# nikitinvv/libtike-cufft

Hardware: AMD Instinct MI355X
Metric: fwd+adj patterns/s (higher is better)
Workload: dtype f32

## Files before the change

libtike-cufft_amd/csrc/adjreg_map.hpp:

```cpp
#pragma once

namespace pty {

constexpr int kBucketPx = 4;

template <int N_, int NT_>
struct AdjRegCfg {
    static constexpr int N = N_, NT = NT_;
    static constexpr int C = 16;
    static constexpr int WC = C + kBucketPx;
    static constexpr int G = NT / WC;
    static constexpr int RPG = (N + G - 2) / (G - 1);
    static constexpr int HW = G * RPG;
    static constexpr int P = WC;
    static constexpr int COL0 = kBucketPx;
    static constexpr int TILE = (N + 2) * P + kBucketPx;
    static constexpr int SG = 1;
    static constexpr int STAGE = SG * RPG * WC;
    static_assert(G >= 2 && HW >= N + RPG, "window too low");
};

struct AdjRegWin {
    int t, X0, Ybase, gb;
};

template <class Cfg>
PTY_FN int adjreg_retire_count(const AdjRegWin& w, int t, int Xa, int sy) {
    const bool fits = t == w.t && Xa >= w.X0 && Xa + Cfg::C < w.X0 + Cfg::WC && sy >= w.Ybase && sy - w.Ybase < Cfg::HW;
    return fits ? (sy - w.Ybase) / Cfg::RPG : Cfg::G;
}

template <class Cfg>
PTY_FN void adjreg_advance(AdjRegWin& w, int nret, int t, int sx, int sy, int x0pad) {
    if (nret >= Cfg::G) {
        w.t = t;
        w.X0 = (sx / kBucketPx) * kBucketPx + x0pad;
        w.Ybase = sy;
        w.gb = 0;
    } else {
        w.Ybase += nret * Cfg::RPG;
        w.gb = (w.gb + nret) % Cfg::G;
    }
}

template <class Cfg>
PTY_FN int adjreg_rank(const AdjRegWin& w, int g) {
    const int k = g - w.gb;
    return k < 0 ? k + Cfg::G : k;
}
template <class Cfg>
PTY_FN int adjreg_row0(const AdjRegWin& w, int g) { return w.Ybase + adjreg_rank<Cfg>(w, g) * Cfg::RPG; }

template <class Cfg>
PTY_FN int adjreg_stage_slot(int rank, int r, int cw) { return (rank * Cfg::RPG + r) * Cfg::WC + cw; }

template <class Cfg>
PTY_FN int adjreg_tile_row(int i) {
    const int r = i + 1;
    return r < 0 ? 0 : (r > Cfg::N + 1 ? Cfg::N + 1 : r);
}

template <class Cfg>
PTY_FN void adjreg_combine(c32* acc, const c32* tile, const AdjRegWin& w, int g, int cw, int Xa, int sy, int pad, float fy, float fx) {
    constexpr int RPG = Cfg::RPG, P = Cfg::P;
    constexpr int B = 4, NB = (RPG + B - 1) / B;
    const float w00 = (1.0f - fx) * (1.0f - fy), w01 = fx * (1.0f - fy);
    const float w10 = (1.0f - fx) * fy, w11 = fx * fy;
    const int i0 = adjreg_row0<Cfg>(w, g) - sy + pad;
    const c32* tp = tile + (cw + Cfg::COL0 - 1 - (Xa - w.X0));
    const c32* tq = tp + adjreg_tile_row<Cfg>(i0 - 1) * P;
    c32 up0 = tq[1], up1 = tq[0];
    c32 t0[2][B], t1[2][B];
    auto request = [&](int b) {
#pragma unroll
        for (int u = 0; u < B; ++u) {
            if (b * B + u < RPG) {
                const c32* tr = tp + adjreg_tile_row<Cfg>(i0 + b * B + u) * P;
                t0[b & 1][u] = tr[1]; t1[b & 1][u] = tr[0];
            }
        }
        asm volatile("" ::: "memory");
    };
    request(0);
#pragma unroll
    for (int b = 0; b < NB; ++b) {
        if (b + 1 < NB) request(b + 1);
#pragma unroll
        for (int u = 0; u < B; ++u) {
            if (b * B + u < RPG) {
                acc[b * B + u] = acc[b * B + u] + (t0[b & 1][u] * w00 + t1[b & 1][u] * w01 + up0 * w10 + up1 * w11);
                up0 = t0[b & 1][u]; up1 = t1[b & 1][u];
            }
        }
    }
}

}
```

libtike-cufft_amd/csrc/k_cols_window.hpp:

```cpp
#pragma once


template <int N>
struct WinCfg {
    static constexpr int C = ColCfg<N>::C;
    static constexpr int WC = C + kBucketPx;
    static constexpr int H = N + 8;
    static constexpr bool fits = (size_t)((N + 2) * (C + 2) + H * WC) * sizeof(c32) <= 160 * 1024;
};

template <int N, bool SPLIT = false, int CW = 0>
__global__ __launch_bounds__(Plan<N>::T * (CW ? CW : ColCfg<N>::C)) void k_cols_adjwin(const ColArgs a, const int seglen) {
    using P = Plan<N>;
    using F = Fft<P, +1>;
    constexpr int E = P::E, T = P::T, C = CW ? CW : ColCfg<N>::C, NT = T * C;
    constexpr int LAST = P::NSTEP - 1;
    constexpr int WC = C + kBucketPx, H = WinCfg<N>::H;
    constexpr int CP = C + 2;
    __shared__ c32 lds[(N + 2) * CP];
    __shared__ c32 win[H * WC];

    const int tid = threadIdx.x;
    const int c = tid % C, j0 = tid / C;
    const int strip = blockIdx.x % a.nstrips, seg = blockIdx.x / a.nstrips;
    const int x0 = (a.strip0 + strip) * C;
    const int x = x0 + c;
    const Geom ge = a.ge;
    const int ix = x - ge.pad;
    const bool col_ok = ix >= 0 && ix < ge.nprb;
    const float cinv = 1.0f / (float)N;
    const c32 zero = c32{0.0f, 0.0f};
    const float det_sc = a.det_acc ? det_scale_of(a.det) : 0.0f;
    auto at = [&](int i) { return (i + 1) * CP + c + 1; };

    F fft;
    fft.init(j0, a.table);
    for (int o = tid; o < H * WC; o += NT) win[o] = zero;
    for (int o = tid; o < (N + 2) * CP; o += NT) lds[o] = zero;

    c32 pr[E];
    int cur_t = -1;
    int t_w = -1, X0 = 0, Ybase = 0, Ytop = 0;

    auto flush = [&](int ya, int yb) {
        if (yb <= ya) return;
        c32* fo = a.dst + (size_t)t_w * ge.nz * ge.n;
        const int cnt = (yb - ya) * WC;
        for (int o = tid; o < cnt; o += NT) {
            const int Y = ya + o / WC, col = o % WC;
            const int slot = (Y % H) * WC + col;
            const c32 v = win[slot];
            win[slot] = zero;
            const int X = X0 + col;
            if ((v.x != 0.0f || v.y != 0.0f) && Y < ge.nz && X >= 0 && X < ge.n) {
                const size_t e = ((size_t)t_w * ge.nz + Y) * ge.n + X;
                accum_c32(a.dst, a.det_acc, det_sc, e, v);
            }
        }
    };

    constexpr int NRG = NT / (C + 1) > 0 ? NT / (C + 1) : 1;
    constexpr int NITEM = (C + 1) * NRG;
    const int rpt = (ge.nprb + 1 + NRG - 1) / NRG;

    const RunBounds rb = run_bounds(a, seg, seglen);
    const int kb = rb.kb, ke = rb.ke;
    __shared__ RunMeta rm;
    load_run(rm, a.order, a.scan, kb, ke, tid);
    auto decode = [&](int k) { return run_decode(rm, k, kb, ke, ge); };
    auto tile_of = [&](const RunSt& st, int k) { return run_tile<N>(a, st.p, k); };

    __syncthreads();
    STAMP_DECL
    RunSt st = decode(kb);
    c32 v[E];
    if (st.have && st.q.valid) {
        const c32* tile_in = tile_of(st, kb);
        if (a.nt & 8)
            fft.template load<(SPLIT ? 1 : 0)>(v, j0, [&](int i) { return __builtin_nontemporal_load(tile_in + (size_t)i * N + x); });
        else
            fft.template load<(SPLIT ? 1 : 0)>(v, j0, [&](int i) { return tile_in[(size_t)i * N + x]; });
    }
    for (int k = kb; k < ke; ++k) {
        RunSt nx = decode(k + 1);
        if (!st.q.valid) {
            if (nx.have && nx.q.valid) {
                const c32* tile_in = tile_of(nx, k + 1);
                fft.template load<(SPLIT ? 1 : 0)>(v, j0, [&](int i) { return tile_in[(size_t)i * N + x]; });
            }
            st = nx;
            continue;
        }
        const Pos q = st.q;
        if (st.t != cur_t) {
            const c32* prb = a.aux + (size_t)st.t * ge.nprb * ge.nprb;
#pragma unroll
            for (int m = 0; m < E; ++m) {
                const int iy = j0 + m * T - ge.pad;
                const bool ok = col_ok && iy >= 0 && iy < ge.nprb;
                const c32 w = prb[ok ? ((size_t)iy * ge.nprb + ix) : 0];
                pr[m] = ok ? w * cinv : zero;
            }
            cur_t = st.t;
        }
        STAMP(0)
        STAMP_DRAIN();
        STAMP(1)
        if (SPLIT) {
            fft.template compute<LAST>(v);
        } else {
        fft.template compute<0>(v);
        if (P::NSTEP > 1) {
            fft.template store<0>(v, j0, [&](int i, c32 val) { lds[at(i)] = val; });
            __syncthreads();
            fft.template load<1>(v, j0, [&](int i) { return lds[at(i)]; });
            if (P::NSTEP > 2) {
                __syncthreads();
                fft.template compute<1>(v);
                fft.template store<1>(v, j0, [&](int i, c32 val) { lds[at(i)] = val; });
                __syncthreads();
                fft.template load<2>(v, j0, [&](int i) { return lds[at(i)]; });
            }
            fft.template compute<LAST>(v);
        }
        }
        {
            c32 nat[E];
            F::to_natural(v, nat);
#pragma unroll
            for (int m = 0; m < E; ++m) {
                const c32 w = pr[m];
                nat[m] = c32{w.x * nat[m].x + w.y * nat[m].y, w.x * nat[m].y - w.y * nat[m].x};
            }
            STAMP(2)
            if (SPLIT) __syncthreads();
            STAMP(3)
#pragma unroll
            for (int m = 0; m < E; ++m) lds[at(j0 + m * T)] = nat[m];
        }
        STAMP(8)
        if (nx.have && nx.q.valid) {
            const c32* tile_in = tile_of(nx, k + 1);
            if (a.nt & 8)
                fft.template load<(SPLIT ? 1 : 0)>(v, j0, [&](int i) { return __builtin_nontemporal_load(tile_in + (size_t)i * N + x); });
            else
                fft.template load<(SPLIT ? 1 : 0)>(v, j0, [&](int i) { return tile_in[(size_t)i * N + x]; });
        }
        STAMP(9)
        const int Xa = q.sx + x0 - ge.pad;
        const bool fitsw = (st.t == t_w) && Xa >= X0 && Xa + C < X0 + WC && q.sy >= Ybase;
        if (!fitsw) {
            __syncthreads();
            flush(Ybase, Ytop);
            t_w = st.t;
            X0 = (q.sx / kBucketPx) * kBucketPx + x0 - ge.pad;
            Ybase = q.sy;
            Ytop = q.sy;
        } else if (q.sy > Ybase) {
            flush(Ybase, q.sy < Ytop ? q.sy : Ytop);
            Ybase = q.sy;
            if (Ytop < Ybase) Ytop = Ybase;
        }
        if (Ytop < q.sy + ge.nprb + 1) Ytop = q.sy + ge.nprb + 1;
        STAMP(4)
        __syncthreads();
        STAMP(5)
        for (int item = tid; item < NITEM; item += NT) {
            const int cc = item % (C + 1), rg = item / (C + 1);
            const int ixo = x0 - ge.pad + cc;
            if (ixo < 0 || ixo > ge.nprb) continue;
            const float w00 = (1.0f - q.fx) * (1.0f - q.fy), w01 = q.fx * (1.0f - q.fy);
            const float w10 = (1.0f - q.fx) * q.fy, w11 = q.fx * q.fy;
            const int y0 = rg * rpt;
            int y1 = y0 + rpt;
            if (y1 > ge.nprb + 1) y1 = ge.nprb + 1;
            if (y0 >= y1) continue;
            const c32* tp = lds + (y0 + ge.pad) * CP + cc;
            c32 up0 = tp[1], up1 = tp[0];
            int slot = (q.sy + y0) % H;
            const int colw = Xa - X0 + cc;
            int yy = y0;
            auto trips = [&](auto uc) {
                constexpr int U = decltype(uc)::value;
                for (; yy + U <= y1; yy += U) {
                    c32 t0[U], t1[U], wv[U];
                    c32* wp[U];
#pragma unroll
                    for (int u = 0; u < U; ++u) {
                        const c32* tq = tp + (u + 1) * CP;
                        int su = slot + u;
                        su = su >= H ? su - H : su;
                        wp[u] = win + su * WC + colw;
                        t0[u] = tq[1]; t1[u] = tq[0];
                    }
#pragma unroll
                    for (int u = 0; u < U; ++u) wv[u] = *wp[u];
#pragma unroll
                    for (int u = 0; u < U; ++u) {
                        *wp[u] = wv[u] + (t0[u] * w00 + t1[u] * w01 + up0 * w10 + up1 * w11);
                        up0 = t0[u]; up1 = t1[u];
                    }
                    tp += U * CP;
                    slot += U;
                    slot = slot >= H ? slot - H : slot;
                }
            };
            trips(std::integral_constant<int, 3>{});
            for (; yy < y1; ++yy) {
                tp += CP;
                const c32 t00 = tp[1], t01 = tp[0];
                win[slot * WC + colw] += t00 * w00 + t01 * w01 + up0 * w10 + up1 * w11;
                up0 = t00; up1 = t01;
                slot = slot + 1 == H ? 0 : slot + 1;
            }
        }
        STAMP(6)
        if (!SPLIT) __syncthreads();
        st = nx;
    }
    __syncthreads();
    flush(Ybase, Ytop);
    STAMP(7)
    STAMP_FLUSH(a.stamps ? a.stamps + 12 : a.stamps)
}

template <int N, bool SPLIT = false>
__global__ __launch_bounds__(Plan<N>::T * ColCfg<N>::C, 2) void k_cols_adjreg(const ColArgs a, const int seglen) {
    using P = Plan<N>;
    using F = Fft<P, +1>;
    constexpr int E = P::E, T = P::T, C = ColCfg<N>::C, NT = T * C;
    constexpr int LAST = P::NSTEP - 1;
    using W = AdjRegCfg<N, NT>;
    static_assert(C == W::C, "strip width");
    constexpr int WC = W::WC, G = W::G, RPG = W::RPG;
    __shared__ c32 lds[W::TILE];
    __shared__ c32 wtab[N];
    __shared__ c32 stage[W::STAGE];

    const int tid = threadIdx.x;
    const int c = tid % C, j0 = tid / C;
    const int cw = tid % WC, g = tid / WC;
    const int strip = blockIdx.x % a.nstrips, seg = blockIdx.x / a.nstrips;
    const int x0 = (a.strip0 + strip) * C;
    const int x = x0 + c;
    const Geom ge = a.ge;
    const int ix = x - ge.pad;
    const bool col_ok = ix >= 0 && ix < ge.nprb;
    const float cinv = 1.0f / (float)N;
    const c32 zero = c32{0.0f, 0.0f};
    const float det_sc = a.det_acc ? det_scale_of(a.det) : 0.0f;
    auto at = [&](int i) { return (i + 1) * W::P + c + W::COL0; };

    F fft;
    for (int o = tid; o < N; o += NT) wtab[o] = a.table[o];
    for (int o = tid; o < W::TILE; o += NT) lds[o] = zero;

    c32 pr[E];
    int cur_t = -1;
    c32 acc[RPG];
#pragma unroll
    for (int r = 0; r < RPG; ++r) acc[r] = zero;
    AdjRegWin w{-1, 0, 0, 0};

    auto add_to_object = [&](const c32 v, int t, int Y, int X) {
        if ((v.x != 0.0f || v.y != 0.0f) && Y < ge.nz && X >= 0 && X < ge.n)
            accum_c32(a.dst, a.det_acc, det_sc, ((size_t)t * ge.nz + Y) * ge.n + X, v);
    };
    auto retire = [&](int nret) {
        if (w.t < 0 || g >= G || adjreg_rank<W>(w, g) >= nret) return;
        const int Y0 = adjreg_row0<W>(w, g), X = w.X0 + cw;
#pragma unroll
        for (int r = 0; r < RPG; ++r) {
            add_to_object(acc[r], w.t, Y0 + r, X);
            acc[r] = zero;
        }
    };
    auto stage_groups = [&](int nret) {
        if (g >= G) return;
        const int rank = adjreg_rank<W>(w, g);
        if (rank >= nret) return;
#pragma unroll
        for (int r = 0; r < RPG; ++r) {
            stage[adjreg_stage_slot<W>(rank, r, cw)] = acc[r];
            acc[r] = zero;
        }
    };

    const RunBounds rb = run_bounds(a, seg, seglen);
    const int kb = rb.kb, ke = rb.ke;
    __shared__ RunMeta rm;
    load_run(rm, a.order, a.scan, kb, ke, tid);
    auto decode = [&](int k) { return run_decode(rm, k, kb, ke, ge); };
    auto tile_of = [&](const RunSt& st, int k) { return run_tile<N>(a, st.p, k); };

    __syncthreads();
    STAMP_DECL
    RunSt st = decode(kb);
    c32 v[E];
    if (st.have && st.q.valid) {
        const c32* tile_in = tile_of(st, kb);
        if (a.nt & 8)
            fft.template load<(SPLIT ? 1 : 0)>(v, j0, [&](int i) { return __builtin_nontemporal_load(tile_in + (size_t)i * N + x); });
        else
            fft.template load<(SPLIT ? 1 : 0)>(v, j0, [&](int i) { return tile_in[(size_t)i * N + x]; });
    }
    for (int k = kb; k < ke; ++k) {
        RunSt nx = decode(k + 1);
        if (!st.q.valid) {
            if (nx.have && nx.q.valid) {
                const c32* tile_in = tile_of(nx, k + 1);
                fft.template load<(SPLIT ? 1 : 0)>(v, j0, [&](int i) { return tile_in[(size_t)i * N + x]; });
            }
            st = nx;
            continue;
        }
        const Pos q = st.q;
        int jz = j0;
        asm volatile("" : "+v"(jz));
        if (st.t != cur_t) {
            const c32* prb = a.aux + (size_t)st.t * ge.nprb * ge.nprb;
#pragma unroll
            for (int m = 0; m < E; ++m) {
                const int iy = j0 + m * T - ge.pad;
                const bool ok = col_ok && iy >= 0 && iy < ge.nprb;
                const c32 pw = prb[ok ? ((size_t)iy * ge.nprb + ix) : 0];
                pr[m] = ok ? pw * cinv : zero;
            }
            cur_t = st.t;
        }
        STAMP(0)
        STAMP_DRAIN();
        STAMP(1)
        if (SPLIT) {
            fft.template init_step<LAST>(jz, wtab);
            fft.template compute<LAST>(v);
        } else {
            fft.template compute<0>(v);
            if (P::NSTEP > 1) {
                fft.template store<0>(v, j0, [&](int i, c32 val) { lds[at(i)] = val; });
                __syncthreads();
                fft.template load<1>(v, j0, [&](int i) { return lds[at(i)]; });
                if (P::NSTEP > 2) {
                    __syncthreads();
                    if constexpr (P::NSTEP > 2) fft.template init_step<1>(jz, wtab);
                    fft.template compute<1>(v);
                    fft.template store<1>(v, j0, [&](int i, c32 val) { lds[at(i)] = val; });
                    __syncthreads();
                    fft.template load<2>(v, j0, [&](int i) { return lds[at(i)]; });
                }
                if constexpr (P::NSTEP > 1) fft.template init_step<LAST>(jz, wtab);
                fft.template compute<LAST>(v);
            }
        }
        {
            c32 nat[E];
            F::to_natural(v, nat);
#pragma unroll
            for (int m = 0; m < E; ++m) {
                const c32 pw = pr[m];
                nat[m] = c32{pw.x * nat[m].x + pw.y * nat[m].y, pw.x * nat[m].y - pw.y * nat[m].x};
            }
            STAMP(2)
            if (SPLIT) __syncthreads();
            STAMP(3)
#pragma unroll
            for (int m = 0; m < E; ++m) lds[at(j0 + m * T)] = nat[m];
        }
        STAMP(8)
        if (nx.have && nx.q.valid) {
            const c32* tile_in = tile_of(nx, k + 1);
            if (a.nt & 8)
                fft.template load<(SPLIT ? 1 : 0)>(v, j0, [&](int i) { return __builtin_nontemporal_load(tile_in + (size_t)i * N + x); });
            else
                fft.template load<(SPLIT ? 1 : 0)>(v, j0, [&](int i) { return tile_in[(size_t)i * N + x]; });
        }
        STAMP(9)
        const int Xa = q.sx + x0 - ge.pad;
        const int nret = adjreg_retire_count<W>(w, st.t, Xa, q.sy);
        const AdjRegWin was = w;
        int nstaged = 0;
        if (nret > 0) {
            if (nret <= W::SG) {
                stage_groups(nret);
                nstaged = nret;
            } else {
                retire(nret);
            }
            adjreg_advance<W>(w, nret, st.t, q.sx, q.sy, x0 - ge.pad);
        }
        STAMP(4)
        __syncthreads();
        STAMP(5)
        for (int o = tid; o < nstaged * RPG * WC; o += NT) add_to_object(stage[o], was.t, was.Ybase + o / WC, was.X0 + o % WC);
        if (g < G) adjreg_combine<W>(acc, lds, w, g, cw, Xa, q.sy, ge.pad, q.fy, q.fx);
        STAMP(6)
        if (!SPLIT) __syncthreads();
        st = nx;
    }
    retire(G);
    STAMP(7)
    STAMP_FLUSH(a.stamps ? a.stamps + 12 : a.stamps)
}

template <int N, int MODE, bool SPLIT = false, int NM = 1, int CW = 0>
__global__ __launch_bounds__(Plan<N>::T * (CW ? CW : ColCfg<N>::C)) void k_cols_gatherwin(const ColArgs a, const int seglen) {
    static_assert(MODE == M_FWD || MODE == M_ADJ_PRB, "forward operator or probe adjoint");
    static_assert(NM == 1 || (MODE == M_FWD && !SPLIT), "several probe modes: un-split forward pass only");
    if (MODE == M_FWD && a.skip && *a.skip != 0.0) return;
    using P = Plan<N>;
    constexpr int DIR = (MODE == M_FWD) ? -1 : +1;
    using F = Fft<P, DIR>;
    constexpr int E = P::E, T = P::T, C = CW ? CW : ColCfg<N>::C, NT = T * C;
    constexpr int LAST = P::NSTEP - 1;
    constexpr int WC = C + kBucketPx, H = WinCfg<N>::H;
    constexpr int R0 = P::radix(0);
    __shared__ c32 lds[SPLIT ? 1 : N * C];
    __shared__ c32 win[(H + 1) * WC];

    const int tid = threadIdx.x;
    const int c = tid % C, j0 = tid / C;
    const int strip = blockIdx.x % a.nstrips, seg = blockIdx.x / a.nstrips;
    const int x0 = (a.strip0 + strip) * C;
    const int x = x0 + c;
    const Geom ge = a.ge;
    const int ix = x - ge.pad;
    const bool col_ok = ix >= 0 && ix < ge.nprb;
    const float cinv = 1.0f / (float)N;
    const c32 zero = c32{0.0f, 0.0f};
    const float det_sc = (MODE == M_ADJ_PRB && a.det_acc) ? det_scale_of(a.det) : 0.0f;

    __shared__ c32 wtab[NM > 1 ? N : 1];
    F fft;
    if (NM == 1) fft.init(j0, a.table);
    else for (int o = tid; o < N; o += NT) wtab[o] = a.table[o];
    for (int o = tid; o < (H + 1) * WC; o += NT) win[o] = zero;

    c32 pr[E];
    c32 prnext[NM > 1 ? E : 1];
    int cur_t = -1;
    auto probe_strip = [&](c32* dst, int km, int t) {
        const c32* prb = (NM == 1 ? a.aux : a.auxm[km]) + (size_t)t * ge.nprb * ge.nprb;
#pragma unroll
        for (int b = 0; b < E / R0; ++b)
#pragma unroll
            for (int tt = 0; tt < R0; ++tt) {
                const int iy = j0 + b * T + tt * (N / R0) - ge.pad;
                const bool ok = col_ok && iy >= 0 && iy < ge.nprb;
                const c32 w = prb[ok ? ((size_t)iy * ge.nprb + ix) : 0];
                dst[b * R0 + tt] = ok ? w * cinv : zero;
            }
    };
    int t_w = -1, X0 = 0, Ylo = 0, Yhi = 0;

    auto flush_probe = [&](int t) {
#pragma unroll
        for (int m = 0; m < E; ++m) {
            const int iy = j0 + m * T - ge.pad;
            if (col_ok && iy >= 0 && iy < ge.nprb) {
                const size_t e = ((size_t)t * ge.nprb + iy) * ge.nprb + ix;
                accum_c32(a.dst, a.det_acc, det_sc, e, pr[m] * cinv);
            }
        }
    };

    const RunBounds rb = run_bounds(a, seg, seglen);
    const int kb = rb.kb, ke = rb.ke;
    __shared__ RunMeta rm;
    load_run(rm, a.order, a.scan, kb, ke, tid);

    struct St { int p, t, Xa; Pos q; bool have; };
    c32 pre_val = zero;
    int pre_slot = -1;
    bool pre_inb = false;
    auto prepare_issue = [&](int k, int kend) -> St {
        St st;
        st.have = k < kend;
        st.p = 0; st.t = 0; st.Xa = 0; st.q = Pos{0, 0, 0.f, 0.f, false, false};
        pre_slot = -1;
        if (!st.have) return st;
        st.p = uni_i(rm.p[k - kb]);
        st.t = st.p / ge.nscan;
        st.q = decode_xy(uni_f(rm.py[k - kb]), uni_f(rm.px[k - kb]), ge);
        if (!st.q.valid) return st;
        const c32* ft = (MODE == M_FWD ? a.src : a.aux) + (size_t)st.t * ge.nz * ge.n;
        st.Xa = st.q.sx + x0 - ge.pad;
        const int Ra = st.q.sy, Rb = st.q.sy + ge.nprb + 1;
        const bool colfit = (st.t == t_w) && st.Xa >= X0 && st.Xa + C < X0 + WC;
        if (!colfit) {
            t_w = st.t;
            X0 = (st.q.sx / kBucketPx) * kBucketPx + x0 - ge.pad;
            Ylo = Ra; Yhi = Ra;
        } else if (Ra < Ylo || Ra > Yhi) {
            Ylo = Ra; Yhi = Ra;
        } else {
            Ylo = Ra;
        }
        if (Rb > Yhi) {
            const int cnt = (Rb - Yhi) * WC;
            if (cnt <= NT) {
                if (tid < cnt) {
                    const int Y = Yhi + tid / WC, col = tid % WC;
                    const int X = X0 + col;
                    const bool inb = Y < ge.nz && X >= 0 && X < ge.n;
                    pre_val = ft[inb ? ((size_t)Y * ge.n + X) : 0];
                    pre_inb = inb;
                    pre_slot = (Y % H) * WC + col;
                }
            } else {
                for (int o = tid; o < cnt; o += NT) {
                    const int Y = Yhi + o / WC, col = o % WC;
                    const int X = X0 + col;
                    const bool inb = Y < ge.nz && X >= 0 && X < ge.n;
                    const c32 val = ft[inb ? ((size_t)Y * ge.n + X) : 0];
                    const int ws = (Y % H) * WC + col;
                    win[ws] = inb ? val : zero;
                    if (ws < WC) win[H * WC + ws] = inb ? val : zero;
                }
            }
            Yhi = Rb;
        }
        return st;
    };
    auto prepare_commit = [&]() {
        if (pre_slot >= 0) {
            const c32 val = pre_inb ? pre_val : zero;
            win[pre_slot] = val;
            if (pre_slot < WC) win[H * WC + pre_slot] = val;
        }
    };
    auto prepare = [&](int k, int kend) -> St {
        St st = prepare_issue(k, kend);
        prepare_commit();
        return st;
    };

    __syncthreads();
    if constexpr (MODE == M_ADJ_PRB) {
        auto decode_only = [&](int k) -> St {
            const RunSt d = run_decode<false>(rm, k, kb, ke, ge);
            return St{d.p, d.t, 0, d.q, d.have};
        };
        auto load_tile = [&](c32* v, const St& st, int k) {
            const c32* tile_in = run_tile<N>(a, st.p, k);
            fft.template load<(SPLIT ? 1 : 0)>(v, j0, [&](int i) { return tile_in[(size_t)i * N + x]; });
        };
        __syncthreads();
        St st = decode_only(kb);
        c32 v[E];
        if (st.have && st.q.valid) load_tile(v, st, kb);
        for (int k = kb; k < ke; ++k) {
            St nx = decode_only(k + 1);
            if (!st.q.valid) {
                if (nx.have && nx.q.valid) load_tile(v, nx, k + 1);
                st = nx;
                continue;
            }
            if (st.t != cur_t) {
                if (cur_t >= 0) flush_probe(cur_t);
#pragma unroll
                for (int m = 0; m < E; ++m) pr[m] = zero;
                cur_t = st.t;
            }
            if (!SPLIT) fft.template compute<0>(v);
            if (!SPLIT && P::NSTEP > 1) {
                fft.template store<0>(v, j0, [&](int i, c32 val) { lds[i * C + c] = val; });
                __syncthreads();
            } else {
                __syncthreads();
            }
            const St cur = prepare_issue(k, ke);
            if (SPLIT) {
                fft.template compute<LAST>(v);
            } else if (P::NSTEP > 1) {
                fft.template load<1>(v, j0, [&](int i) { return lds[i * C + c]; });
                if (P::NSTEP > 2) {
                    __syncthreads();
                    fft.template compute<1>(v);
                    fft.template store<1>(v, j0, [&](int i, c32 val) { lds[i * C + c] = val; });
                    __syncthreads();
                    fft.template load<2>(v, j0, [&](int i) { return lds[i * C + c]; });
                }
                fft.template compute<LAST>(v);
            }
            c32 nat[E];
            F::to_natural(v, nat);
            if (nx.have && nx.q.valid) load_tile(v, nx, k + 1);
            prepare_commit();
            __syncthreads();
            const Pos q = cur.q;
            const float w00 = (1.0f - q.fx) * (1.0f - q.fy), w01 = q.fx * (1.0f - q.fy);
            const float w10 = (1.0f - q.fx) * q.fy, w11 = q.fx * q.fy;
            const int colw = cur.Xa - X0 + c;
            int slot = (q.sy + j0 - ge.pad + 2 * H) % H;
#pragma unroll
            for (int m = 0; m < E; ++m) {
                const int iy = j0 + m * T - ge.pad;
                const bool ok = col_ok && iy >= 0 && iy < ge.nprb;
                const c32* r0 = win + slot * WC + colw;
                const c32 patch = r0[0] * w00 + r0[1] * w01 + r0[WC] * w10 + r0[WC + 1] * w11;
                const c32 term = cmulc(nat[m], patch);
                pr[m] += ok ? term : zero;
                slot += T;
                slot = slot >= H ? slot - H : slot;
            }
            st = nx;
        }
        if (cur_t >= 0) flush_probe(cur_t);
    } else {
        St st = prepare(kb, ke);
        __syncthreads();
        STAMP_DECL
        for (int k = kb; k < ke; ++k) {
            if (NM > 1 || st.t != cur_t) {
                probe_strip(pr, 0, st.t);
                cur_t = st.t;
            }
            if (!st.q.valid) {
#pragma unroll
                for (int km = 0; km < NM; ++km) {
                    c32* tile_out = (NM == 1 ? a.dst : a.dstm[km]) + (size_t)st.p * N * N;
#pragma unroll
                    for (int m = 0; m < E; ++m) tile_out[(size_t)(j0 + m * T) * N + x] = zero;
                }
                __syncthreads();
                st = prepare(k + 1, ke);
                __syncthreads();
                continue;
            }
            const Pos q = st.q;
            const float w00 = (1.0f - q.fx) * (1.0f - q.fy), w01 = q.fx * (1.0f - q.fy);
            const float w10 = (1.0f - q.fx) * q.fy, w11 = q.fx * q.fy;
            const int colw = st.Xa - X0 + c;
            const int slot0 = (q.sy + j0 - ge.pad + 2 * H) % H;
            auto patch_at = [&](int slot) {
                const c32* r0 = win + slot * WC + colw;
                return r0[0] * w00 + r0[1] * w01 + r0[WC] * w10 + r0[WC + 1] * w11;
            };

            c32 v[E];
            c32 vbase[NM > 1 ? E : 1];
            St nx;
            {
                STAMP(0)
                c32 nat[E];
                int slot = slot0;
#pragma unroll
                for (int m = 0; m < E; ++m) {
                    nat[m] = patch_at(slot);
                    slot += T;
                    slot = slot >= H ? slot - H : slot;
                }
                F::from_natural(nat, v);
#ifdef PTY_STAMPS
                asm volatile("s_waitcnt lgkmcnt(0)" ::: "memory");
#pragma unroll
                for (int s2 = 0; s2 < E; ++s2) asm volatile("" : "+v"(v[s2]));
#endif
                STAMP(1)
                if (NM > 1) {
#pragma unroll
                    for (int s2 = 0; s2 < E; ++s2) vbase[s2] = v[s2];
                }
#pragma unroll
                for (int s2 = 0; s2 < E; ++s2) v[s2] = cmul(pr[s2], v[s2]);
            }
            fft.template compute<0>(v);
            if (SPLIT) {
                c32* tile_out = a.dst + (size_t)st.p * N * N;
#ifdef PTY_STAMPS
#pragma unroll
                for (int s2 = 0; s2 < E; ++s2) asm volatile("" : "+v"(v[s2]));
#endif
                STAMP(2)
                fft.template store<0>(v, j0, [&](int i, c32 val) { tile_out[(size_t)i * N + x] = val; });
                STAMP(3)
                __syncthreads();
                STAMP(4)
                nx = prepare_issue(k + 1, ke);
                prepare_commit();
                STAMP(5)
                __syncthreads();
                STAMP(6)
                st = nx;
                continue;
            }
            int jz = j0;
            if (NM > 1) asm volatile("" : "+v"(jz));
#pragma unroll
            for (int km = 0; km < NM; ++km) {
                if (NM > 1) {
                    if (km > 0) {
#pragma unroll
                        for (int s2 = 0; s2 < E; ++s2) v[s2] = cmul(prnext[s2], vbase[s2]);
                        fft.template compute<0>(v);
                    }
                    if (km + 1 < NM) probe_strip(prnext, km + 1, st.t);
                }
                if (P::NSTEP > 1) {
                    STAMP(2)
                    fft.template store<0>(v, j0, [&](int i, c32 val) { lds[i * C + c] = val; });
                    STAMP(3)
                    __syncthreads();
                    STAMP(4)
                    if (km == 0) nx = prepare_issue(k + 1, ke);
                    fft.template load<1>(v, j0, [&](int i) { return lds[i * C + c]; });
                    if (P::NSTEP > 2) {
                        __syncthreads();
                        if constexpr (NM > 1 && P::NSTEP > 2) fft.template init_step<1>(jz, wtab);
                        fft.template compute<1>(v);
                        fft.template store<1>(v, j0, [&](int i, c32 val) { lds[i * C + c] = val; });
                        __syncthreads();
                        fft.template load<2>(v, j0, [&](int i) { return lds[i * C + c]; });
                    }
                    if constexpr (NM > 1 && P::NSTEP > 1) fft.template init_step<LAST>(jz, wtab);
                    fft.template compute<LAST>(v);
                } else if (km == 0) {
                    __syncthreads();
                    nx = prepare_issue(k + 1, ke);
                }
                STAMP(5)
                c32* tile_out = (NM == 1 ? a.dst : a.dstm[km]) + (size_t)st.p * N * N;
                if (a.nt & 4)
                    fft.template store<LAST>(v, j0, [&](int i, c32 val) { __builtin_nontemporal_store(val, tile_out + (size_t)i * N + x); });
                else
                    fft.template store<LAST>(v, j0, [&](int i, c32 val) { tile_out[(size_t)i * N + x] = val; });
// ... 138 lines not shown
```

libtike-cufft_amd/csrc/k_rows.hpp:

```cpp
#pragma once

template <bool WGSYNC, bool TWLDS, class P, int DIR, class Put, class Get>
__device__ __forceinline__ void row_steps(Fft<P, DIR>& fft, c32* v, const int j0, Put put, Get get, const int jz = 0,
                                          const c32* wtab = nullptr) {
    constexpr int T = P::T, LAST = P::NSTEP - 1;
    fft.template compute<0>(v);
    if constexpr (P::NSTEP > 1) {
        fft.template store<0>(v, j0, put);
        row_sync<T, WGSYNC>();
        fft.template load<1>(v, j0, get);
        if constexpr (P::NSTEP > 2) {
            row_sync<T, WGSYNC>();
            if constexpr (TWLDS) fft.template init_step<1>(jz, wtab);
            fft.template compute<1>(v);
            fft.template store<1>(v, j0, put);
            row_sync<T, WGSYNC>();
            fft.template load<2>(v, j0, get);
        }
        if constexpr (TWLDS) fft.template init_step<LAST>(jz, wtab);
        fft.template compute<LAST>(v);
    }
}

template <int N, int DIR>
__global__ __launch_bounds__(256) void k_rows(const RowArgs a) {
    using P = Plan<N>;
    using F = Fft<P, DIR>;
    using L = RowLds<N>;
    constexpr int E = P::E, T = P::T, B = 256 / T;
    constexpr int LAST = P::NSTEP - 1;
    __shared__ c32 lds[P::NSTEP > 1 ? B * L::FS : 1];

    const int tid = threadIdx.x;
    const int f = tid / T, j0 = tid % T;
    F fft;
    fft.init(j0, a.table);
    const c32 zero = c32{0.0f, 0.0f};
    const long long nb = (a.nrows + B - 1) / B;
    for (long long batch = blockIdx.x; batch < nb; batch += gridDim.x) {
        const long long r = batch * B + f;
        const bool ok = r < a.nrows;
        const long long tile = r / N;
        const c32* srow = a.src + (size_t)((a.tile_index && ok) ? (long long)a.tile_index[tile] : tile) * N * N + (size_t)(r % N) * N;
        c32* drow = a.dst + ((a.dst_indexed && a.tile_index && ok)
                                 ? (size_t)a.tile_index[tile] * N * N + (size_t)(r % N) * N
                                 : (size_t)r * N);
        c32 v[E];
        if (a.nt & 1)
            fft.template load<0>(v, j0, [&](int i) { return (ok && i >= a.xa && i < a.xb) ? __builtin_nontemporal_load(srow + i) : zero; });
        else
            fft.template load<0>(v, j0, [&](int i) { return (ok && i >= a.xa && i < a.xb) ? srow[i] : zero; });
        fft.template compute<0>(v);
        if (P::NSTEP > 1) {
            fft.template store<0>(v, j0, [&](int i, c32 val) { lds[L::at(f, i)] = val; });
            row_sync<T>();
            fft.template load<1>(v, j0, [&](int i) { return lds[L::at(f, i)]; });
            if (P::NSTEP > 2) {
                row_sync<T>();
                fft.template compute<1>(v);
                fft.template store<1>(v, j0, [&](int i, c32 val) { lds[L::at(f, i)] = val; });
                row_sync<T>();
                fft.template load<2>(v, j0, [&](int i) { return lds[L::at(f, i)]; });
            }
            fft.template compute<LAST>(v);
        }
        if (a.nt & 2)
            fft.template store<LAST>(v, j0, [&](int i, c32 val) {
                if (ok && i >= a.wa && i < a.wb) __builtin_nontemporal_store(val, drow + i);
            });
        else
            fft.template store<LAST>(v, j0, [&](int i, c32 val) {
                if (ok && i >= a.wa && i < a.wb) drow[i] = val;
            });
        if (P::NSTEP > 1) row_sync<T>();
    }
}

template <int N, int DIR>
__global__ __launch_bounds__(256) void k_rows_split(const RowArgs a) {
    static_assert(N == 256, "split row pass is written for the 16 x 16 plan");
    using P = Plan<N>;
    using F = Fft<P, DIR>;
    using L = RowLds<N>;
    constexpr int E = P::E, T = P::T, B = 256 / T;
    constexpr int LAST = P::NSTEP - 1;
    __shared__ c32 lds[B * L::FS];

    const int tid = threadIdx.x;
    const int f = tid / T, j0 = tid % T;
    F fft;
    fft.init(j0, a.table);
    auto put = [&](int i, c32 val) { lds[L::at(f, i)] = val; };
    auto get = [&](int i) { return lds[L::at(f, i)]; };
    const c32 zero = c32{0.0f, 0.0f};
    const long long nitems = (a.nrows / N) * 16;
    for (long long item = blockIdx.x; item < nitems; item += gridDim.x) {
        const long long tile = item / 16;
        const int jp = (int)(item % 16);
        const long long stile = a.tile_index ? (long long)a.tile_index[tile] : tile;
        const c32* sbase = a.src + (size_t)stile * N * N;
        c32* dbase = a.dst + (size_t)((a.dst_indexed && a.tile_index) ? stile : tile) * N * N;
        c32 v[E];
        if (DIR < 0) {
            const int x = tid;
            const bool colok = x >= a.xa && x < a.xb;
#pragma unroll
            for (int t = 0; t < 16; ++t) {
                const c32 val = __builtin_nontemporal_load(sbase + (size_t)(jp + 16 * t) * N + x);
                v[t] = colok ? val : zero;
            }
#pragma unroll
            for (int t = 1; t < 16; ++t) v[t] = cmul(v[t], a.table[(jp * t) & (N - 1)]);
            fft_reg<16, -1>(v);
#pragma unroll
            for (int t = 0; t < 16; ++t) lds[L::at(t, x)] = v[brev(t, 4)];
            __syncthreads();
            fft.template load<0>(v, j0, get);
            row_steps<false, false>(fft, v, j0, put, get);
            c32* drow = dbase + (size_t)(jp + 16 * f) * N;
            fft.template store<LAST>(v, j0, [&](int i, c32 val) { __builtin_nontemporal_store(val, drow + i); });
            __syncthreads();
        } else {
            const c32* srow = sbase + (size_t)(jp + 16 * f) * N;
            fft.template load<0>(v, j0, [&](int i) { return __builtin_nontemporal_load(srow + i); });
            fft.template compute<0>(v);
            fft.template store<0>(v, j0, put);
            row_sync<T>();
            fft.template load<1>(v, j0, get);
            fft.template compute<LAST>(v);
            row_sync<T>();
            fft.template store<LAST>(v, j0, put);
            __syncthreads();
            const int x = tid;
#pragma unroll
            for (int t = 0; t < 16; ++t) v[t] = lds[L::at(t, x)];
            fft_reg<16, +1>(v);
            if (x >= a.wa && x < a.wb) {
#pragma unroll
                for (int k1 = 0; k1 < 16; ++k1)
                    __builtin_nontemporal_store(v[brev(k1, 4)], dbase + (size_t)(16 * jp + k1) * N + x);
            }
            __syncthreads();
        }
    }
}

__device__ __forceinline__ float fsqrt(float x) { return __builtin_amdgcn_sqrtf(x); }
__device__ __forceinline__ float frcp(float x) { return __builtin_amdgcn_rcpf(x); }
__device__ __forceinline__ float flog2(float x) { return __builtin_amdgcn_logf(x); }
constexpr float kLn2 = 0.693147180559945309f;
enum CgModel { MODEL_GAUSSIAN = 0, MODEL_POISSON_ML = 1 };
__device__ __forceinline__ c32 pml_shift(const c32 d, const c32 dl) {
    return d - dl * c32{flog2(d.x + 1e-32f), flog2(d.y + 1e-32f)};
}
__device__ __forceinline__ c32 pml_term(const c32 x, const c32 dl, const c32 c) {
    const c32 ax = c32{fabsf(x.x), fabsf(x.y)};
    return (ax - c) - dl * c32{flog2(ax.x + 1e-32f), flog2(ax.y + 1e-32f)};
}
template <bool PML>
struct TrialTerm {
    c32 sd, dl, c;
    __device__ __forceinline__ explicit TrialTerm(const c32 d) {
        if constexpr (PML) {
            dl = d * kLn2;
            c = pml_shift(d, dl);
        } else {
            sd = c32{fsqrt(d.x), fsqrt(d.y)};
        }
    }
    __device__ __forceinline__ c32 operator()(const c32 x) const {
        if constexpr (PML) {
            return pml_term(x, dl, c);
        } else {
            const c32 df = c32{fsqrt(fabsf(x.x)), fsqrt(fabsf(x.y))} - sd;
            return df * df;
        }
    }
};

__device__ __forceinline__ c32 load_masked(const c32* __restrict__ p, unsigned m) {
    const c32 val = __builtin_nontemporal_load(p);
    return c32{__uint_as_float(__float_as_uint(val.x) & m), __uint_as_float(__float_as_uint(val.y) & m)};
}
__device__ __forceinline__ float load_masked(const float* __restrict__ p, unsigned m) {
    return __uint_as_float(__float_as_uint(__builtin_nontemporal_load(p)) & m);
}

enum RowEp { EP_STATS = 1, EP_PROJECT = 2, EP_LINESEARCH = 3, EP_CROSS = 6, EP_LINESEARCH_M = 7, EP_STATS_M = 8 };
constexpr int kMaxModes = 8;
constexpr int kMaxCand = 16;
constexpr int kLsGroupsRows = 7;

struct RowFusedArgs {
    const c32* s1;
    const c32* s2;
    c32* out;
    const float* data;
    const c32* table;
    long long nrows;
    double* sums;
    const double* ab;
    float gamma0;
    int ncand;
    int xa, xb;
    const float* inten;
    float* acc1;
    int first;
    const c32* sm[2 * kMaxModes];
    int nmodes;
    c32* ip;
    double* st;
    const double* gamma_dev;
    double* maxword;
    FoldBuf fold;
    int overwrite;
    int decide, decide_which, decide_gamma_word, decide_next;
    unsigned long long* best_zero;
    int nbest;
    const unsigned* mask;
};

__device__ inline void ls_decide_dev(double* __restrict__ st, const int which, const int gamma_word, const int next_ngroups) {
    if (st[PTYCHO_ST_LS_RESOLVED] != 0.0) return;
    const int ngroups = (int)st[PTYCHO_ST_LS_NGROUPS];
    const int ncand = (int)st[PTYCHO_ST_LS_NCAND];
    int tried = (int)st[PTYCHO_ST_LS_TRIED];
    double step = st[PTYCHO_ST_LS_GAMMA0];
    bool done = false;
    for (int grp = 0; grp < ngroups && !done; ++grp) {
        const double* c = st + PTYCHO_ST_COSTS + grp * (kMaxCand + 1);
        const float fp1 = (float)c[ncand];
        for (int j = 0; j < ncand; ++j) {
            if (!((float)c[j] > fp1)) {
                st[gamma_word] = 0.5 * step;
                st[PTYCHO_ST_HINT + which] = (double)(tried + j);
                done = true;
                break;
            }
            if (step < 1e-32) {
                st[gamma_word] = 0.0;
                st[PTYCHO_ST_HINT + which] = 14.0;
                st[PTYCHO_ST_LS_FAILED] += 1.0;
                done = true;
                break;
            }
            step *= 0.5;
        }
        if (!done) tried += ncand;
    }
    if (!done && next_ngroups == 0) {
        st[gamma_word] = 0.0;
        st[PTYCHO_ST_LS_FAILED] += 1.0;
        done = true;
    }
    st[PTYCHO_ST_LS_RESOLVED] = done ? 1.0 : 0.0;
    st[PTYCHO_ST_LS_TRIED] = (double)tried;
    st[PTYCHO_ST_LS_GAMMA0] = step;
    st[PTYCHO_ST_LS_NCAND] = (double)kMaxCand;
    st[PTYCHO_ST_LS_NGROUPS] = (double)next_ngroups;
}


template <int N, int EP>
constexpr int fused_min_waves() {
    if (!is_pow2(N)) return 1;
    return (N <= 512 && (EP == EP_LINESEARCH || EP == EP_LINESEARCH_M || EP == EP_PROJECT || EP == EP_CROSS)) ? 2
           : (N == 512 && (EP == EP_STATS || EP == EP_STATS_M)) ? 3 : 1;
}
template <>
constexpr int fused_min_waves<256, EP_STATS>() { return 4;
}
template <int N>
__global__ __launch_bounds__(256) void k_pack_mask(const unsigned char* __restrict__ m, unsigned* __restrict__ out,
                                                   unsigned* __restrict__ nmeasured) {
    using P = Plan<N>;
    static_assert(P::E <= 32, "one mask word per thread and row");
    const int w = blockIdx.x * 256 + threadIdx.x;
    if (w >= N * P::T) return;
    const int y = w / P::T, j0 = w % P::T;
    unsigned bits = 0u;
    for (int k = 0; k < P::E; ++k) bits |= (m[y * N + j0 + k * P::T] != 0 ? 1u : 0u) << k;
    out[w] = bits;
    if (bits) atomicAdd(nmeasured, (unsigned)__popc(bits));
}
__device__ __forceinline__ unsigned mask_bit(unsigned w, int k) { return (unsigned)((int)(w << (31 - k)) >> 31); }
__device__ __forceinline__ float and_f(float x, unsigned m) { return __uint_as_float(__float_as_uint(x) & m); }
__device__ __forceinline__ c32 and_c(c32 x, unsigned m) { return c32{and_f(x.x, m), and_f(x.y, m)}; }

template <int N, int EP, bool FW = false, bool MASK = false, int MODEL = MODEL_GAUSSIAN>
// ... 395 lines not shown
```

Measured before the change: 1.704 million.

## Stage split column-pass tiles into LDS ring via direct global-to-LDS loads

For the split adjoint column kernel, tiles are now fetched with global_load_lds_dwordx4 into a per-wave LDS ring and read back in FFT order, with the next tile's request issued right after the read. This replaces per-thread strided global loads, and a lighter waitcnt-plus-barrier replaces __syncthreads. The split path now runs compute<0> instead of the last step, drops the LDS twiddle table, and the row kernel gains an explicit twiddle multiply via readlane. A host-side checker validates the ring mapping. The inline asm that manipulates m0 is fragile, and the changed split FFT step order alters numerics structure.

```diff
diff --git a/libtike-cufft_amd/csrc/adjreg_map.hpp b/libtike-cufft_amd/csrc/adjreg_map.hpp
--- a/libtike-cufft_amd/csrc/adjreg_map.hpp
+++ b/libtike-cufft_amd/csrc/adjreg_map.hpp
@@ -95,4 +95,29 @@
     }
 }
 
+template <int N_>
+struct AdjRingCfg {
+    static constexpr int N = N_, C = 16, E = 16, T = N / E;
+    static constexpr int WAVE = 64, NW = T * C / WAVE;
+    static constexpr int JW = WAVE / C;
+    static constexpr int PIECES = 8;
+    static constexpr int PIECE = WAVE * 2;
+    static constexpr int SEG = PIECES * PIECE;
+    static constexpr int RING = NW * SEG;
+    static constexpr int ROW_STEP = (WAVE / 8 / JW) * T;
+    static_assert(RING == N * C && SEG == JW * E * C, "the ring holds one strip tile");
+};
+
+template <class R>
+PTY_FN int adjring_src_row(int wave, int i, int lane) {
+    const int rr = 8 * i + lane / 8;
+    return wave * R::JW + rr % R::JW + (rr / R::JW) * R::T;
 }
+template <class R>
+PTY_FN int adjring_src_col(int lane) { return 2 * (lane % 8); }
+template <class R>
+PTY_FN int adjring_dst_slot(int wave, int i, int lane) { return wave * R::SEG + i * R::PIECE + 2 * lane; }
+template <class R>
+PTY_FN int adjring_read_slot(int tid, int m) { return (tid / R::WAVE) * R::SEG + m * R::WAVE + tid % R::WAVE; }
+
+}
diff --git a/libtike-cufft_amd/csrc/host_adjdma.cpp b/libtike-cufft_amd/csrc/host_adjdma.cpp
--- /dev/null
+++ b/libtike-cufft_amd/csrc/host_adjdma.cpp
@@ -0,0 +1,65 @@
+#include <cstdint>
+#include <cstdio>
+#include <vector>
+
+#include "fft_core.hpp"
+#include "adjreg_map.hpp"
+
+using namespace pty;
+
+template <int N, int ST>
+static bool check(const char* name) {
+    using P = Plan<N>;
+    using F = Fft<P, +1>;
+    using R = AdjRingCfg<N>;
+    constexpr int C = R::C, NT = P::T * C;
+    static_assert(P::E == R::E && P::T == R::T, "the ring is cut for the plan's threads");
+    long long bad = 0;
+    const size_t scratch_base = 4096;
+    for (int strip = 0; strip < N / C; ++strip) {
+        const int x0 = strip * C;
+        std::vector<int> ring(R::RING, -1);
+        std::vector<int> requested(N * C, 0);
+        for (int wave = 0; wave < R::NW; ++wave)
+            for (int i = 0; i < R::PIECES; ++i)
+                for (int lane = 0; lane < R::WAVE; ++lane) {
+                    const int row = adjring_src_row<R>(wave, i, lane), col = adjring_src_col<R>(lane);
+                    const int slot = adjring_dst_slot<R>(wave, i, lane);
+                    if (row < 0 || row >= N || col < 0 || col + 1 >= C) { ++bad; continue; }
+                    const size_t src = scratch_base + ((size_t)row * N + x0 + col) * sizeof(c32);
+                    if (src % 16 != 0) ++bad;
+                    if (row != adjring_src_row<R>(wave, 0, lane) + i * R::ROW_STEP) ++bad;
+                    if (slot != wave * R::SEG + i * R::PIECE + 2 * lane) ++bad;
+                    if (slot < wave * R::SEG || slot + 1 >= (wave + 1) * R::SEG) { ++bad; continue; }
+                    for (int e = 0; e < 2; ++e) {
+                        if (ring[slot + e] != -1) ++bad;
+                        ring[slot + e] = row * C + col + e;
+                        ++requested[row * C + col + e];
+                    }
+                }
+        for (int e = 0; e < N * C; ++e)
+            if (requested[e] != 1) ++bad;
+        for (int tid = 0; tid < NT; ++tid) {
+            const int c = tid % C, j0 = tid / C;
+            F fft;
+            c32 rows[P::E];
+            fft.template load<ST>(rows, j0, [&](int i) { return c32{(float)i, 0.0f}; });
+            for (int m = 0; m < P::E; ++m) {
+                const int slot = adjring_read_slot<R>(tid, m);
+                if (slot < (tid / R::WAVE) * R::SEG || slot >= (tid / R::WAVE + 1) * R::SEG) { ++bad; continue; }
+                if (ring[slot] != (int)rows[m].x * C + c) ++bad;
+            }
+        }
+    }
+    std::printf("N=%d %s waves=%d requests=%d segment=%zu B ring=%zu B row_step=%d bad=%lld %s\n", N, name, R::NW, R::PIECES,
+                (size_t)R::SEG * sizeof(c32), (size_t)R::RING * sizeof(c32), R::ROW_STEP, bad, bad == 0 ? "ok" : "BAD");
+    return bad == 0;
+}
+
+int main() {
+    bool ok = true;
+    ok = check<256, 1>("split") && ok;
+    ok = check<256, 0>("unsplit") && ok;
+    std::printf("%s\n", ok ? "OK" : "FAIL");
+    return ok ? 0 : 1;
+}
diff --git a/libtike-cufft_amd/csrc/k_cols_window.hpp b/libtike-cufft_amd/csrc/k_cols_window.hpp
--- a/libtike-cufft_amd/csrc/k_cols_window.hpp
+++ b/libtike-cufft_amd/csrc/k_cols_window.hpp
@@ -11,6 +11,7 @@
 
 template <int N, bool SPLIT = false, int CW = 0>
 __global__ __launch_bounds__(Plan<N>::T * (CW ? CW : ColCfg<N>::C)) void k_cols_adjwin(const ColArgs a, const int seglen) {
+    static_assert(!SPLIT || N == 256, "split column pass is written for the 16 x 16 plan");
     using P = Plan<N>;
     using F = Fft<P, +1>;
     constexpr int E = P::E, T = P::T, C = CW ? CW : ColCfg<N>::C, NT = T * C;
@@ -107,7 +108,7 @@
         STAMP_DRAIN();
         STAMP(1)
         if (SPLIT) {
-            fft.template compute<LAST>(v);
+            fft.template compute<0>(v);
         } else {
         fft.template compute<0>(v);
         if (P::NSTEP > 1) {
@@ -233,8 +234,12 @@
     using W = AdjRegCfg<N, NT>;
     static_assert(C == W::C, "strip width");
     constexpr int WC = W::WC, G = W::G, RPG = W::RPG;
-    __shared__ c32 lds[W::TILE];
-    __shared__ c32 wtab[N];
+    static_assert(!SPLIT || N == 256, "split column pass is written for the 16 x 16 plan");
+    using R = AdjRingCfg<N>;
+    constexpr int RINGN = SPLIT ? R::RING : 0;
+    __shared__ __attribute__((aligned(SPLIT ? 16 : 8))) c32 ring_tile[RINGN + W::TILE];
+    c32* const lds = ring_tile + RINGN;
+    __shared__ c32 wtab[SPLIT ? 1 : N];
     __shared__ c32 stage[W::STAGE];
 
     const int tid = threadIdx.x;
@@ -252,8 +257,36 @@
     auto at = [&](int i) { return (i + 1) * W::P + c + W::COL0; };
 
     F fft;
-    for (int o = tid; o < N; o += NT) wtab[o] = a.table[o];
+    if constexpr (!SPLIT) {
+        for (int o = tid; o < N; o += NT) wtab[o] = a.table[o];
+    }
     for (int o = tid; o < W::TILE; o += NT) lds[o] = zero;
+
+    const int lane = tid % R::WAVE, wave = uni_i(tid / R::WAVE);
+    const unsigned ring_m0 = (unsigned)(size_t)ring_tile + (unsigned)(wave * R::SEG * (int)sizeof(c32));
+    const unsigned ring_voff =
+        (unsigned)((adjring_src_row<R>(wave, 0, lane) * N + x0 + adjring_src_col<R>(lane)) * (int)sizeof(c32));
+    const int ring_rd = adjring_read_slot<R>(tid, 0);
+    auto ring_request = [&](const c32* tile_in) {
+#pragma unroll
+        for (int i = 0; i < R::PIECES; ++i) {
+            const c32* sb = tile_in + (size_t)i * R::ROW_STEP * N;
+            const unsigned dst = ring_m0 + (unsigned)(i * R::PIECE * (int)sizeof(c32));
+            unsigned keep;
+            asm volatile("s_mov_b32 %0, m0\n\ts_mov_b32 m0, %3\n\ts_nop 0\n\tglobal_load_lds_dwordx4 %1, %2\n\ts_mov_b32 m0, %0"
+                         : "=&s"(keep) : "v"(ring_voff), "s"(sb), "s"(dst) : "memory");
+        }
+    };
+    auto ring_read = [&](c32* v) {
+#pragma unroll
+        for (int m = 0; m < E; ++m) v[m] = ring_tile[ring_rd + m * R::WAVE];
+        asm volatile("s_waitcnt lgkmcnt(0)" ::: "memory");
+    };
+    auto ring_barrier = [&]() {
+        asm volatile("s_waitcnt lgkmcnt(0)" ::: "memory");
+        __builtin_amdgcn_s_barrier();
+        asm volatile("" ::: "memory");
+    };
 
     c32 pr[E];
     int cur_t = -1;
@@ -299,17 +332,22 @@
     c32 v[E];
     if (st.have && st.q.valid) {
         const c32* tile_in = tile_of(st, kb);
-        if (a.nt & 8)
-            fft.template load<(SPLIT ? 1 : 0)>(v, j0, [&](int i) { return __builtin_nontemporal_load(tile_in + (size_t)i * N + x); });
-        else
-            fft.template load<(SPLIT ? 1 : 0)>(v, j0, [&](int i) { return tile_in[(size_t)i * N + x]; });
+        if constexpr (SPLIT) {
+            ring_request(tile_in);
+        } else {
+            if (a.nt & 8)
+                fft.template load<0>(v, j0, [&](int i) { return __builtin_nontemporal_load(tile_in + (size_t)i * N + x); });
+            else
+                fft.template load<0>(v, j0, [&](int i) { return tile_in[(size_t)i * N + x]; });
+        }
     }
     for (int k = kb; k < ke; ++k) {
         RunSt nx = decode(k + 1);
         if (!st.q.valid) {
             if (nx.have && nx.q.valid) {
                 const c32* tile_in = tile_of(nx, k + 1);
-                fft.template load<(SPLIT ? 1 : 0)>(v, j0, [&](int i) { return tile_in[(size_t)i * N + x]; });
+                if constexpr (SPLIT) ring_request(tile_in);
+                else fft.template load<0>(v, j0, [&](int i) { return tile_in[(size_t)i * N + x]; });
             }
             st = nx;
             continue;
@@ -329,12 +367,16 @@
             cur_t = st.t;
         }
         STAMP(0)
-        STAMP_DRAIN();
-        STAMP(1)
-        if (SPLIT) {
-            fft.template init_step<LAST>(jz, wtab);
-            fft.template compute<LAST>(v);
+        if constexpr (SPLIT) {
+            asm volatile("s_waitcnt vmcnt(0)" ::: "memory");
+            STAMP(1)
+            ring_read(v);
+            if (nx.have && nx.q.valid) ring_request(tile_of(nx, k + 1));
+            STAMP(9)
+            fft.template compute<0>(v);
         } else {
+            STAMP_DRAIN();
+            STAMP(1)
             fft.template compute<0>(v);
             if (P::NSTEP > 1) {
                 fft.template store<0>(v, j0, [&](int i, c32 val) { lds[at(i)] = val; });
@@ -361,20 +403,22 @@
                 nat[m] = c32{pw.x * nat[m].x + pw.y * nat[m].y, pw.x * nat[m].y - pw.y * nat[m].x};
             }
             STAMP(2)
-            if (SPLIT) __syncthreads();
+            if constexpr (SPLIT) ring_barrier();
             STAMP(3)
 #pragma unroll
             for (int m = 0; m < E; ++m) lds[at(j0 + m * T)] = nat[m];
         }
         STAMP(8)
-        if (nx.have && nx.q.valid) {
-            const c32* tile_in = tile_of(nx, k + 1);
-            if (a.nt & 8)
-                fft.template load<(SPLIT ? 1 : 0)>(v, j0, [&](int i) { return __builtin_nontemporal_load(tile_in + (size_t)i * N + x); });
-            else
-                fft.template load<(SPLIT ? 1 : 0)>(v, j0, [&](int i) { return tile_in[(size_t)i * N + x]; });
-        }
-        STAMP(9)
+        if constexpr (!SPLIT) {
+            if (nx.have && nx.q.valid) {
+                const c32* tile_in = tile_of(nx, k + 1);
+                if (a.nt & 8)
+                    fft.template load<0>(v, j0, [&](int i) { return __builtin_nontemporal_load(tile_in + (size_t)i * N + x); });
+                else
+                    fft.template load<0>(v, j0, [&](int i) { return tile_in[(size_t)i * N + x]; });
+            }
+            STAMP(9)
+        }
         const int Xa = q.sx + x0 - ge.pad;
         const int nret = adjreg_retire_count<W>(w, st.t, Xa, q.sy);
         const AdjRegWin was = w;
@@ -389,7 +433,8 @@
             adjreg_advance<W>(w, nret, st.t, q.sx, q.sy, x0 - ge.pad);
         }
         STAMP(4)
-        __syncthreads();
+        if constexpr (SPLIT) ring_barrier();
+        else __syncthreads();
         STAMP(5)
         for (int o = tid; o < nstaged * RPG * WC; o += NT) add_to_object(stage[o], was.t, was.Ybase + o / WC, was.X0 + o % WC);
         if (g < G) adjreg_combine<W>(acc, lds, w, g, cw, Xa, q.sy, ge.pad, q.fy, q.fx);
@@ -431,8 +476,8 @@
 
     __shared__ c32 wtab[NM > 1 ? N : 1];
     F fft;
-    if (NM == 1) fft.init(j0, a.table);
-    else for (int o = tid; o < N; o += NT) wtab[o] = a.table[o];
+    if (NM > 1) for (int o = tid; o < N; o += NT) wtab[o] = a.table[o];
+    else if (!SPLIT) fft.init(j0, a.table);
     for (int o = tid; o < (H + 1) * WC; o += NT) win[o] = zero;
 
     c32 pr[E];
@@ -570,7 +615,7 @@
             }
             const St cur = prepare_issue(k, ke);
             if (SPLIT) {
-                fft.template compute<LAST>(v);
+                fft.template compute<0>(v);
             } else if (P::NSTEP > 1) {
                 fft.template load<1>(v, j0, [&](int i) { return lds[i * C + c]; });
                 if (P::NSTEP > 2) {
diff --git a/libtike-cufft_amd/csrc/k_rows.hpp b/libtike-cufft_amd/csrc/k_rows.hpp
--- a/libtike-cufft_amd/csrc/k_rows.hpp
+++ b/libtike-cufft_amd/csrc/k_rows.hpp
@@ -122,6 +122,7 @@
             __syncthreads();
         } else {
             const c32* srow = sbase + (size_t)(jp + 16 * f) * N;
+            const c32 wl = cconj(a.table[(jp * (tid & 15)) & (N - 1)]);
             fft.template load<0>(v, j0, [&](int i) { return __builtin_nontemporal_load(srow + i); });
             fft.template compute<0>(v);
             fft.template store<0>(v, j0, put);
@@ -135,6 +136,14 @@
 #pragma unroll
             for (int t = 0; t < 16; ++t) v[t] = lds[L::at(t, x)];
             fft_reg<16, +1>(v);
+            if (jp != 0) {
+#pragma unroll
+                for (int k1 = 0; k1 < 16; ++k1) {
+                    const c32 w = c32{__int_as_float(__builtin_amdgcn_readlane(__float_as_int(wl.x), k1)),
+                                      __int_as_float(__builtin_amdgcn_readlane(__float_as_int(wl.y), k1))};
+                    v[brev(k1, 4)] = cmul(v[brev(k1, 4)], w);
+                }
+            }
             if (x >= a.wa && x < a.wb) {
 #pragma unroll
                 for (int k1 = 0; k1 < 16; ++k1)
```

Result: faster. 1.737 million, median of 6 (+1.9%).
